# RuyiLian/CheckerPose

Hardware: AMD Instinct MI355X
Metric: crops/sec forward (256x256, npt=512) (higher is better)
Workload: dtype bf16; 1 GPU; LMO 'ape' hr18GNN2_res6_gnn3Skip_mlpQuery npt=512, PoseNet_GNNskip forward, deterministic random-init weights; global_batch=256, parallelism=dp1 (no forward collective), launch=hipGraph replay of 104 kernel launches

## Files before the change

### __graft_entry__.py

```python
import os
import subprocess
import sys

ROOT = os.path.dirname(os.path.abspath(__file__))
if ROOT not in sys.path:
    sys.path.insert(0, ROOT)


def build():
    csrc = os.path.join(ROOT, "checkerpose_amd", "csrc")
    subprocess.check_call(["make", "-C", csrc, "-j4", "ARCH=gfx950"])
    import checkerpose_amd
    from checkerpose_amd import _abi
    lib = _abi.load()
    assert lib.cp_version() >= 232


def smoke():
    import torch
    from oracle import checkerpose_oracle as O
    from checkerpose_amd.synthetic import build_net, det_image
    oracle_kwargs = lambda: dict(backbone="hrnet_w18", res_log2=6, init_n_graph=2, n_graph=3, local_k=2, slope=0.01,
                                 graph_slope=0.2, init_graph_slope=0.2)
    assert torch.cuda.is_available(), "smoke() needs an MI355X"
    torch.set_grad_enabled(False)
    net = build_net(seed=1)
    img = det_image(1, seed=0)
    ref, _ = O.posenet_forward(net.state_dict(), img, net.init_net.knn_idx, 512, **oracle_kwargs())
    net = net.cuda()
    out = net(img.cuda(), None)
# ... 15 lines not shown
```

### checkerpose_amd/_abi.py

```python
import ctypes as C
import os

_HERE = os.path.dirname(os.path.abspath(__file__))
LIB_PATH = os.environ.get("CHECKERPOSE_AMD_LIB") or os.path.join(_HERE, "libcheckerpose_hip.so")

CP_F32, CP_BF16, CP_F16 = 0, 1, 2
ACT_NONE, ACT_RELU, ACT_LEAKY = 0, 1, 2
LOSS_BCE, LOSS_L1 = 0, 1
POSE_ERR_ADD, POSE_ERR_ADI = 1, 2
BOP_ERR_MSSD, BOP_ERR_MSPD, BOP_ERR_PROJ, BOP_MAP_SMALL, BOP_MAP_LARGE = 1, 2, 4, 16, 32
BOP_MATCH_NO_LDS, BOP_MATCH_SCRATCH_MASK, BOP_SCORES_NO_LDS = 1, 2, 1


class CpConvDesc(C.Structure):
    _fields_ = [("dtype", C.c_int32), ("out_f32", C.c_int32), ("B", C.c_int32), ("H", C.c_int32), ("W", C.c_int32),
                ("Cin", C.c_int32), ("in_cstride", C.c_int32), ("in_coff", C.c_int32),
                ("R", C.c_int32), ("S", C.c_int32), ("stride", C.c_int32), ("pad", C.c_int32),
                ("Ho", C.c_int32), ("Wo", C.c_int32), ("Cout", C.c_int32), ("act", C.c_int32), ("slope", C.c_float), ("ksplit", C.c_int32),
                ("o_base", C.c_int64), ("o_sb", C.c_int64), ("o_sy", C.c_int64), ("o_sx", C.c_int64),
                ("o_sc", C.c_int64)]


_P, _I, _F, _L = C.c_void_p, C.c_int, C.c_float, C.c_longlong

# ... 68 lines not shown

SIGNATURES = {
    "cp_version": (_I, []),
    "cp_device_status": (_I, [_P, _I]),
    "cp_set_deterministic": (None, [_I]),
    "cp_get_deterministic": (_I, []),
    "cp_strerror": (C.c_char_p, [_I]),
    "cp_last_kernel": (C.c_char_p, []),
    "cp_kernel_log_begin": (None, []),
    "cp_kernel_log": (C.c_char_p, []),
    "cp_chan_align": (_I, [_I]),
    "cp_packed_weight_bytes": (C.c_size_t, [_I, _I, _I, _I, _I]),
    "cp_pack_conv_weight": (_I, [_P, _I, _P, _I, _I, _I, _I, _I, _I, _I, _P, _I, _P]),
    "cp_conv2d_igemm": (_I, [_P, C.POINTER(CpConvDesc), _P, _P, _P, _P, _P, _P]),
    "cp_conv2d_igemm_splitk": (_I, [_I, C.c_longlong, _I, _I]),
    "cp_packed_halo_weight_bytes": (C.c_size_t, [_I, _I, _I]),
    "cp_pack_conv3x3_halo_weight": (_I, [_P, _I, _P, _I, _I, _I, _P]),
    "cp_conv3x3_halo": (_I, [_P, C.POINTER(CpConvDesc), _P, _P, _P, _P, _P, _P]),
    "cp_conv2x2_halo_supported": (_I, [_I, _I, _I, _I]),
    "cp_packed_conv2x2_halo_weight_bytes": (C.c_size_t, [_I, _I, _I]),
    "cp_pack_conv2x2_halo_weight": (_I, [_P, _I, _P, _I, _I, _I, _P]),
    "cp_conv2x2_halo": (_I, [_P, C.POINTER(CpConvDesc), _P, _P, _P, _P, _P, _P]),
    "cp_conv3x3_s2_small_supported": (_I, [_I, _I, _I, _I]),
    "cp_conv3x3_s2_small_weight_bytes": (C.c_size_t, [_I, _I]),
    "cp_pack_conv3x3_s2_small_weight": (_I, [_P, _P, _I, _I, _I, _I, _P]),
    "cp_conv3x3_s2_small": (_I, [_P, C.POINTER(CpConvDesc), _P, _P, _P, _P, _P]),
    "cp_conv3x3_halo_up2x_supported": (_I, [_I, _I]),
    "cp_conv3x3_halo_up2x": (_I, [_P, C.POINTER(CpConvDesc), _P, _P, _P, _P, _P]),
    "cp_conv3x3_halo_seg_supported": (_I, [_I, _I, _I]),
    "cp_conv3x3_halo_seg": (_I, [_P, C.POINTER(CpConvDesc), _P, _P, _P, _P, _P, _P, _P, _I, _P]),
# ... 270 lines not shown
```

### checkerpose_amd/csrc/api.hip

```cpp
#include <stdarg.h>
#include <stdio.h>
#include <string.h>

#include "common.h"

extern "C" int cp_version(void) { return 232; }

std::atomic<int> g_cp_deterministic{0};
extern "C" void cp_set_deterministic(int on) { g_cp_deterministic.store(on ? 1 : 0, std::memory_order_relaxed); }
extern "C" int cp_get_deterministic(void) { return g_cp_deterministic.load(std::memory_order_relaxed); }

static std::atomic<uint32_t*> g_status_word[256];
uint32_t* cp_status_word(bool create) {
  const int dev = cp_current_device();
  if (dev < 0 || dev > 255) return nullptr;
  uint32_t* p = g_status_word[dev].load(std::memory_order_acquire);
  if (p || !create) return p;
  hipStreamCaptureStatus cs = hipStreamCaptureStatusNone;
  if (hipStreamIsCapturing(nullptr, &cs) == hipSuccess && cs != hipStreamCaptureStatusNone) return nullptr;
  uint32_t* q = nullptr;
  if (hipMalloc((void**)&q, 256) != hipSuccess) return nullptr;
  if (hipMemset(q, 0, 256) != hipSuccess) { (void)hipFree(q); return nullptr; }
  uint32_t* expect = nullptr;
  if (!g_status_word[dev].compare_exchange_strong(expect, q, std::memory_order_acq_rel)) { (void)hipFree(q); return expect; }
// ... 24 lines not shown
  const size_t have = strlen(g_kernel_log);
  if (have + n + 4 < sizeof(g_kernel_log))
    snprintf(g_kernel_log + have, sizeof(g_kernel_log) - have, "%s%s", have ? " + " : "", g_last_kernel);
}
extern "C" const char* cp_last_kernel(void) { return g_last_kernel; }
extern "C" void cp_kernel_log_begin(void) { g_kernel_log[0] = 0; }
extern "C" const char* cp_kernel_log(void) { return g_kernel_log; }

extern "C" const char* cp_strerror(int code) {
  switch (code) {
    case CP_OK: return "ok";
    case CP_ERR_INVALID: return "invalid argument or unsupported shape";
    case CP_ERR_HIP: return "HIP runtime error (kernel launch / graph call failed)";
    case CP_ERR_ALIGN: return "pointer, channel count or stride not aligned to 16 bytes / 4 channels";
    case CP_ERR_RANGE: return "buffer exceeds 2 GiB 32-bit buffer addressing";
    default: return "unknown checkerpose_hip error code";
  }
}

extern "C" int cp_graph_begin_capture(cp_stream_t stream) {
  return hipStreamBeginCapture((hipStream_t)stream, hipStreamCaptureModeThreadLocal) == hipSuccess ? CP_OK : CP_ERR_HIP;
}

extern "C" int cp_graph_end_capture(cp_stream_t stream, void** graph_exec_out) {
  if (!graph_exec_out) return CP_ERR_INVALID;
  hipGraph_t graph = nullptr;
  if (hipStreamEndCapture((hipStream_t)stream, &graph) != hipSuccess || !graph) return CP_ERR_HIP;
  hipGraphExec_t exec = nullptr;
  hipError_t e = hipGraphInstantiate(&exec, graph, nullptr, nullptr, 0);
  (void)hipGraphDestroy(graph);
// ... 15 lines not shown
```

### checkerpose_amd/csrc/conv_igemm.hip

```cpp
#include <stdlib.h>

#include "common.h"

struct ConvParams {
  const void* in; const void* w; const float* scale; const float* shift; const void* res; void* out;
  int M, H, W, HoWo, Wo;
  int Cin, in_cs, in_coff;
  int R, S, stride, pad;
  int KC, Cout, n_tiles, m_blocks, n_blocks, old_map;
  int act; float slope; int out_f32; int epi_lds;
  uint32_t in_bytes, w_bytes;
  long long o_base, o_sb, o_sy, o_sx, o_sc;
};

template <typename Tag> struct Mma;
template <> struct Mma<F32Tag> {
  static __device__ __forceinline__ void run(const u32x4& w, const u32x4& a, f32x4& acc) {
    acc = __builtin_amdgcn_mfma_f32_16x16x4f32(__uint_as_float(w.x), __uint_as_float(a.x), acc, 0, 0, 0);
    acc = __builtin_amdgcn_mfma_f32_16x16x4f32(__uint_as_float(w.y), __uint_as_float(a.y), acc, 0, 0, 0);
    acc = __builtin_amdgcn_mfma_f32_16x16x4f32(__uint_as_float(w.z), __uint_as_float(a.z), acc, 0, 0, 0);
    acc = __builtin_amdgcn_mfma_f32_16x16x4f32(__uint_as_float(w.w), __uint_as_float(a.w), acc, 0, 0, 0);
  }
};
template <> struct Mma<BF16Tag> {
  static __device__ __forceinline__ void run(const u32x4& w, const u32x4& a, f32x4& acc) {
    acc = __builtin_amdgcn_mfma_f32_16x16x32_bf16(__builtin_bit_cast(bf16x8, w), __builtin_bit_cast(bf16x8, a), acc, 0, 0, 0);
  }
};

template <> struct Mma<F16Tag> {
  static __device__ __forceinline__ void run(const u32x4& w, const u32x4& a, f32x4& acc) { acc = cp_mma16<true>(w, a, acc); }
};

template <typename Tag, int MT, int NT>
__global__ __launch_bounds__(256) void conv_igemm_kernel(const ConvParams p) {
  if (p.out_f32 == 2 || Tag::dtype == CP_F16) cp_f16_saturate_on();
  constexpr int E = Tag::E;
  constexpr int KCH = 4 * E;
  constexpr int ES = 16 / E;
  const int lane = threadIdx.x & 63;
  const int wave = __builtin_amdgcn_readfirstlane(threadIdx.x >> 6);
  const int x = lane & 15, q = lane >> 4;
  const int label = blockIdx.x & 7, slot = blockIdx.x >> 3;
  int nblk = slot % p.n_blocks;
  int mblk = (slot / p.n_blocks) * 8 + label;
  if (p.old_map) { const int m8 = (p.m_blocks + 7) / 8 * 8; mblk = blockIdx.x % m8; nblk = blockIdx.x / m8; }
  if (mblk >= p.m_blocks) return;
  const int m_wave = mblk * (4 * MT * 16) + wave * (MT * 16);
  const int nt0 = nblk * NT;

  int iy0[MT], ix0[MT], rowbase[MT];
#pragma unroll
  for (int mt = 0; mt < MT; ++mt) {
    const int m = m_wave + mt * 16 + x;
    const bool ok = m < p.M;
    const int mm = ok ? m : 0;
    const int b = mm / p.HoWo;
    const int rem = mm - b * p.HoWo;
    const int oy = rem / p.Wo;
    const int ox = rem - oy * p.Wo;
    iy0[mt] = ok ? oy * p.stride - p.pad : -(1 << 28);
// ... 218 lines not shown
        for (int j = 0; j < 4; ++j) {
          if (n + j >= p.Cout) continue;
          const long long o = pix[mt] + (long long)(n + j) * p.o_sc;
          float y = v[j];
          if (p.res) y += f32io ? ((const float*)p.res)[o] : bf16_bits_to_f32(((const uint16_t*)p.res)[o]);
          y = cp_act_apply(y, cp_act_slope(p.act, p.slope));
          if (f32io) ((float*)p.out)[o] = y;
          else if (h16out) ((uint16_t*)p.out)[o] = (uint16_t)f32_to_f16_bits_sat(y);
          else ((uint16_t*)p.out)[o] = (uint16_t)f32_to_bf16_bits(y);
        }
      }
    }
  }
}

template <typename Tag, int NT, int KS>
__global__ __launch_bounds__(KS * 64) void conv_igemm_splitk_kernel(const ConvParams p) {
  if (p.out_f32 == 2 || Tag::dtype == CP_F16) cp_f16_saturate_on();
  constexpr int E = Tag::E, KCH = 4 * E, ES = 16 / E, MT = 2, T = MT * NT;
  constexpr int U = NT == 1 ? 8 : (NT == 2 ? 6 : 4);
  __shared__ __attribute__((aligned(16))) float red[KS * T * 64 * 4];
  const int lane = threadIdx.x & 63;
  const int wave = __builtin_amdgcn_readfirstlane(threadIdx.x >> 6);
  const int x = lane & 15, q = lane >> 4;
  const int nblk = blockIdx.x % p.n_blocks, mblk = blockIdx.x / p.n_blocks;
  const int m0 = mblk * (MT * 16), nt0 = nblk * NT;

  int iy0[MT], ix0[MT], rowbase[MT];
#pragma unroll
  for (int mt = 0; mt < MT; ++mt) {
// ... 167 lines not shown
  cp_mark_kernel("conv_igemm_kernel<%s, %d, %d>", Tag::dtype == CP_BF16 ? "BF16Tag" : (Tag::dtype == CP_F16 ? "F16Tag" : "F32Tag"), MT, NT);
  hipLaunchKernelGGL((conv_igemm_kernel<Tag, MT, NT>), grid, dim3(256), lds, st, p);
}

template <typename Tag, int MT>
static void dispatch_nt(const ConvParams& p, int NT, hipStream_t st) {
  switch (NT) {
    case 1: launch<Tag, MT, 1>(p, st); break;
    case 2: launch<Tag, MT, 2>(p, st); break;
    case 3: launch<Tag, MT, 3>(p, st); break;
    case 4: launch<Tag, MT, 4>(p, st); break;
    default: launch<Tag, MT, 5>(p, st); break;
  }
}

extern "C" int cp_conv2d_igemm(cp_stream_t stream, const CpConvDesc* d, const void* in, const void* packed_w,
                               const float* scale, const float* shift, const void* residual, void* out) {
  if (!d || !in || !packed_w || !scale || !shift || !out) return CP_ERR_INVALID;
  if ((d->dtype != CP_F32 && d->dtype != CP_BF16 && d->dtype != CP_F16) || !cp_act_ok(d->act, d->slope)) return CP_ERR_INVALID;
  const bool halfish = d->dtype == CP_F16 || d->out_f32 == 2;
  if (d->out_f32 < 0 || d->out_f32 > 2 || (d->out_f32 == 2 && d->dtype != CP_BF16) || (halfish && residual)) return CP_ERR_INVALID;
  const int E = cp_chan_align(d->dtype), es = cp_elem_size(d->dtype);
  if (d->B <= 0 || d->H <= 0 || d->W <= 0 || d->Ho <= 0 || d->Wo <= 0 || d->R <= 0 || d->S <= 0 || d->stride <= 0)
    return CP_ERR_INVALID;
  if (d->Cin <= 0 || d->Cin % E || d->in_coff % E || d->in_cstride % E || d->in_coff + d->Cin > d->in_cstride)
    return CP_ERR_ALIGN;
  if (d->Cout <= 0 || (d->o_sc == 1 && d->Cout % 4)) return CP_ERR_ALIGN;
  if (!cp_aligned16(in) || !cp_aligned16(packed_w) || !cp_aligned16(scale) || !cp_aligned16(shift))
    return CP_ERR_ALIGN;
  const long long in_bytes = (long long)d->B * d->H * d->W * d->in_cstride * es;
  if (in_bytes >= (1LL << 31)) return CP_ERR_RANGE;
  const long long M = (long long)d->B * d->Ho * d->Wo;
  if (M >= (1LL << 31)) return CP_ERR_RANGE;
  if (d->o_sc == 1) {
    const int oes = d->out_f32 == 1 ? 4 : es;
    if ((d->o_base % 4) || (d->o_sb % 4) || (d->o_sy % 4) || (d->o_sx % 4)) return CP_ERR_ALIGN;
    if (((uintptr_t)out % (4 * oes)) || (residual && ((uintptr_t)residual % (4 * oes)))) return CP_ERR_ALIGN;
  }
  ConvParams p;
  p.in = in; p.w = packed_w; p.scale = scale; p.shift = shift; p.res = residual; p.out = out;
  p.M = (int)M; p.H = d->H; p.W = d->W; p.HoWo = d->Ho * d->Wo; p.Wo = d->Wo;
  p.Cin = d->Cin; p.in_cs = d->in_cstride; p.in_coff = d->in_coff;
  p.R = d->R; p.S = d->S; p.stride = d->stride; p.pad = d->pad;
  const int K = d->R * d->S * d->Cin, KCH = 4 * E;
  p.KC = (K + KCH - 1) / KCH;
  p.Cout = d->Cout; p.n_tiles = (d->Cout + 15) / 16;
  p.act = d->act; p.slope = d->slope; p.out_f32 = d->out_f32;
  p.in_bytes = (uint32_t)in_bytes;
  p.w_bytes = (uint32_t)((size_t)p.n_tiles * p.KC * 1024);
  p.o_base = d->o_base; p.o_sb = d->o_sb; p.o_sy = d->o_sy; p.o_sx = d->o_sx; p.o_sc = d->o_sc;

  int nts = 1;
  if (const int ks = d->ksplit == -1 ? 0 : splitk_plan(d->dtype, M, p.KC, p.n_tiles, &nts)) {
    hipStream_t st_ = (hipStream_t)stream;
    const bool hin = d->dtype == CP_F16;
    if (ks == 8) { if (nts == 3) launch_splitk<3, 8>(p, st_, hin); else if (nts == 2) launch_splitk<2, 8>(p, st_, hin); else launch_splitk<1, 8>(p, st_, hin); }
    else         { if (nts == 3) launch_splitk<3, 4>(p, st_, hin); else if (nts == 2) launch_splitk<2, 4>(p, st_, hin); else launch_splitk<1, 4>(p, st_, hin); }
    return cp_check_launch();
  }
  int NT = 1, best = 1 << 30;
  for (int nt = 5; nt >= 1; --nt) {
    const int padded = (p.n_tiles + nt - 1) / nt * nt;
    if (padded < best) { best = padded; NT = nt; }
  }
  const long long blocks4 = ((M + 255) / 256) * ((p.n_tiles + NT - 1) / NT);
  int MT = (blocks4 >= 512 && p.KC > 4) ? 4 : 2;
  if (const char* e = cp_knob("CP_CONV_MT")) MT = atoi(e) == 2 ? 2 : 4;
  const int oes_ = d->out_f32 == 1 ? 4 : es;
  const int cpl = 16 / oes_;
  p.epi_lds = (MT == 2 && d->o_sc == 1 && !d->out_f32 && !halfish && (NT == 1 || NT == 2 || NT == 4) && d->Cout % cpl == 0 && d->o_base % cpl == 0 &&
               d->o_sb % cpl == 0 && d->o_sy % cpl == 0 && d->o_sx % cpl == 0 && ((uintptr_t)out % 16) == 0 &&
               (!residual || ((uintptr_t)residual % 16) == 0) && !cp_knob("CP_NO_EPI_LDS")) ? 1 : 0;
  hipStream_t st = (hipStream_t)stream;
  if (d->dtype == CP_F32) { if (MT == 4) dispatch_nt<F32Tag, 4>(p, NT, st); else dispatch_nt<F32Tag, 2>(p, NT, st); }
  else if (d->dtype == CP_F16) { if (MT == 4) dispatch_nt<F16Tag, 4>(p, NT, st); else dispatch_nt<F16Tag, 2>(p, NT, st); }
  else                    { if (MT == 4) dispatch_nt<BF16Tag, 4>(p, NT, st); else dispatch_nt<BF16Tag, 2>(p, NT, st); }
  return cp_check_launch();
}
```

### checkerpose_amd/engine.py

```python
import ctypes as C
import os

import torch

from . import _abi
from ._abi import ACT_LEAKY, ACT_NONE, ACT_RELU, CP_BF16, CP_F16, CP_F32, CpChainTail, CpChainTailConv, CpConvDesc, CpFuseConv

_TORCH_DT = {CP_F32: torch.float32, CP_BF16: torch.bfloat16}
USE_HALO = os.environ.get("CHECKERPOSE_AMD_HALO", "1") != "0"
USE_FUSED_BN = os.environ.get("CHECKERPOSE_AMD_FUSED_BN", "1") != "0"
USE_FUSED_BB = os.environ.get("CHECKERPOSE_AMD_FUSED_BB", "1") != "0"
USE_GEMM = os.environ.get("CHECKERPOSE_AMD_GEMM", "1") != "0"
USE_CHAIN = os.environ.get("CHECKERPOSE_AMD_CHAIN", "1") != "0"
USE_UP_FUSED = os.environ.get("CHECKERPOSE_AMD_UP_FUSED", "1") != "0"
USE_FUSE_OUT = os.environ.get("CHECKERPOSE_AMD_FUSE_OUT", "1") != "0"
USE_S2_SMALL = os.environ.get("CHECKERPOSE_AMD_S2_SMALL", "1") != "0"
USE_SEG_FUSED = os.environ.get("CHECKERPOSE_AMD_SEG_FUSED", "1") != "0"
USE_HALO2 = os.environ.get("CHECKERPOSE_AMD_HALO2", "1") != "0"
USE_CHAIN_TAILS = os.environ.get("CHECKERPOSE_AMD_CHAIN_TAILS", "1") != "0"
USE_CHAIN_TAIL = os.environ.get("CHECKERPOSE_AMD_CHAIN_TAIL", "1") != "0"
FUSE_OUT_MIN_BATCH = int(os.environ.get("CHECKERPOSE_AMD_FUSE_OUT_MIN_BATCH", "1"))
USE_MLP_FUSED = os.environ.get("CHECKERPOSE_AMD_MLP_FUSED", "1") != "0"
MLP_FUSED_MIN_ROWS = int(os.environ.get("CHECKERPOSE_AMD_MLP_FUSED_MIN_ROWS", "1"))
EDGE_SCHED = os.environ.get("CHECKERPOSE_AMD_EDGE_SCHED", "1") != "0"
USE_SPLITK = os.environ.get("CHECKERPOSE_AMD_SPLITK", "1") != "0"
GEMM_WS_SMALL_K = os.environ.get("CHECKERPOSE_AMD_GEMM_WS_SMALL_K", "1") != "0"
USE_MLP_GATHER = os.environ.get("CHECKERPOSE_AMD_MLP_GATHER", "1") != "0"
USE_PATCH_GATHER = os.environ.get("CHECKERPOSE_AMD_PATCH_GATHER", "1") != "0"
USE_STEM = os.environ.get("CHECKERPOSE_AMD_STEM", "1") != "0"
STEM_MIN_BATCH = int(os.environ.get("CHECKERPOSE_AMD_STEM_MIN_BATCH", "96"))
USE_EDGE_FUSED = os.environ.get("CHECKERPOSE_AMD_EDGE_FUSED", "1") != "0"
USE_GNN_F16 = os.environ.get("CHECKERPOSE_AMD_GNN_F16", "1") != "0"
USE_EDGE_TILED = os.environ.get("CHECKERPOSE_AMD_EDGE_TILED", "1") != "0"
EDGE_FUSED_MIN_BATCH = int(os.environ.get("CHECKERPOSE_AMD_EDGE_FUSED_MIN_BATCH", "96"))
CHAIN_MIN_BATCH = int(os.environ.get("CHECKERPOSE_AMD_CHAIN_MIN_BATCH", "40"))
NO_RECYCLE = os.environ.get("CHECKERPOSE_AMD_NO_RECYCLE", "0") == "1"
DTYPES = {"fp32": CP_F32, "f32": CP_F32, "float32": CP_F32, "bf16": CP_BF16, "bfloat16": CP_BF16}


class _ConvLog(list):
# ... 213 lines not shown
        return self._nmarks

    def wait(self, token, dst):
        assert self._open is not None
        self.ops.append(("__wait__", token, dst))

    def par_end(self):
        assert self._open is not None
        self.ops.append(("__join__",))
        self.regions.append((self._open - 1, len(self.ops) - 1))
        self._open = None
        self.lane = 0

    def conv(self, x: Act, wkey, w, scale, shift, R, S, stride, pad, Cout, act=ACT_NONE, slope=0.0, residual: Act = None,
             out: Act = None, transposed=0, phase=0, row_map=None, cout_rows=None, out_f32=False, ostr=None,
             out_tbuf=None, out_hw=None, w_shape=None, out_half=False, in_half=False):
        if out_half or in_half:
            assert self.dtype == CP_BF16 and residual is None and not (out_half and out_f32)
        E = self.E
        wCout, wCin = (w.shape[1], w.shape[0]) if transposed else (w.shape[0], w.shape[1])
        rows = cout_rows if cout_rows is not None else wCout
        if wCin != x.C:
            raise RuntimeError("conv %s: weight expects %d input channels, activation has %d" % (wkey, wCin, x.C))
        halo = (USE_HALO and R == 3 and S == 3 and stride == 1 and pad == 1 and ostr is None and not out_f32
                and not transposed and row_map is None and x.W >= 16 and x.H >= 8 and not (out_half or in_half))
        cdt = CP_F16 if in_half else self.dtype
        if halo and wCout <= 80 and self.dtype == CP_F32:
            halo = _rup(x.Cphys, 16) <= 1.15 * x.Cphys
        kmin = 16 * self.E if not (self.dtype == CP_BF16 and residual is None and x.B * x.H * x.W >= 16384 and GEMM_WS_SMALL_K) else 64
        gemm = (USE_GEMM and R == 1 and S == 1 and stride == 1 and pad == 0 and ostr is None and not out_f32
                and not transposed and row_map is None and wCout >= 96 and x.Cphys >= kmin and not out_half)
        s2small = (USE_S2_SMALL and self.dtype == CP_BF16 and R == 3 and S == 3 and stride == 2 and pad == 1 and ostr is None and not out_f32
                   and not transposed and row_map is None and residual is None and x.H % 2 == 0 and x.W % 2 == 0 and x.B >= self.chain_min
                   and not (out_half or in_half) and bool(self.lib.cp_conv3x3_s2_small_supported(x.H, x.W, x.Cphys, _rup(wCout, self.E))))
        halo2 = (USE_HALO2 and self.dtype == CP_BF16 and R == 2 and S == 2 and stride == 1 and pad == 1 and ostr is None and not out_f32
                 and not transposed and row_map is None and not in_half and not self.ws.repacks_every_step
                 and bool(self.lib.cp_conv2x2_halo_supported(self.dtype, x.H, x.W, _rup(wCout, self.E))))
        if (self.splitk and not transposed and row_map is None and (halo or gemm or s2small or halo2)
                and self.lib.cp_conv2d_igemm_splitk(cdt, x.B * ((x.H + 2 * pad - R) // stride + 1) * ((x.W + 2 * pad - S) // stride + 1),
                                                    R * S * x.Cphys, _rup(wCout, self.E))):
            halo = gemm = s2small = halo2 = False
        if s2small:
            packed = self.ws._pack(("s2small", wkey, x.Cphys), self.lib.cp_conv3x3_s2_small_weight_bytes(x.Cphys, _rup(wCout, self.E)), w,
                                   lambda st, wp, op: self.lib.cp_pack_conv3x3_s2_small_weight(st, wp, wCout, wCin, x.Cphys, _rup(wCout, self.E), op),
                                   "cp_pack_conv3x3_s2_small_weight(%s)" % wkey)
            halo = gemm = False
        elif halo2:
            packed = self.ws._pack(("halo2", wkey, x.Cphys), self.lib.cp_packed_conv2x2_halo_weight_bytes(self.dtype, wCout, x.Cphys), w,
                                   lambda st, wp, op: self.lib.cp_pack_conv2x2_halo_weight(st, self.dtype, wp, wCout, wCin, x.Cphys, op),
                                   "cp_pack_conv2x2_halo_weight(%s)" % wkey)
        elif halo:
            packed = self.ws.pack_halo(wkey, w, wCout, wCin, x.Cphys)
        elif gemm:
            packed = self.ws.pack_gemm(wkey, w, wCout, wCin, x.Cphys, **({"dtype": CP_F16} if in_half else {}))
        else:
            packed = self.ws.pack(wkey, w, wCout, wCin, R, S, x.Cphys, rows, transposed, phase, row_map, **({"dtype": CP_F16} if in_half else {}))
# ... 21 lines not shown
        if residual is not None and ostr is None:
            assert (residual.cstride, residual.coff, residual.H, residual.W) == (out.cstride, out.coff, out.H, out.W), \
                "residual must share the output layout"
        fn = self.lib.cp_conv3x3_halo if halo else (self.lib.cp_gemm_rows if gemm else self.lib.cp_conv2d_igemm)
        if halo2:
            fn = self.lib.cp_conv2x2_halo
        dref = C.byref(d)
        pw, ps, pt = packed.data_ptr(), sc.data_ptr(), sh.data_ptr()
        xtb = x.tbuf
        if halo:
            fam = "conv3x3_halo_s" if wCout <= 80 else ("conv3x3_halo4" if wCout % 256 == 0 else "conv3x3_halo")
        else:
            fam = "gemm_rows" if gemm else "conv_igemm"
        if halo2:
            fam = "conv3x3_halo_s"
        if s2small:
            fam = "conv3x3_s2_small"
            self._add(self.lib.cp_conv3x3_s2_small, lambda P: (dref, P(xtb), pw, ps, pt, P(otb)), fam + ":" + wkey, [xtb], [otb])
        else:
            self._add(fn, lambda P: (dref, P(xtb), pw, ps, pt, P(rtb) if rtb is not None else None, P(otb)),
                      fam + ":" + wkey, [xtb, rtb], [otb])
        fl = 2 * x.B * Ho * Wo * R * S * wCin * wCout
        self.flops += fl
        oes = 4 if out_f32 else self.es
        nbytes = (x.B * x.H * x.W * wCin * self.es + x.B * Ho * Wo * wCout * oes * (2 if residual is not None else 1)
                  + R * S * wCin * wCout * self.es)
        self.conv_log.append((wkey, x.B * Ho * Wo, wCout, R * S * wCin, fl, fam, nbytes))
        return out

    def would_splitk(self, M, K, Cout):
        return bool(self.splitk and self.lib.cp_conv2d_igemm_splitk(self.dtype, M, K, _rup(Cout, self.E)))

    def can_conv_up2x(self, H, W, Cout):
        return (USE_UP_FUSED and 2 * H >= 8 and 2 * W >= 16 and
                bool(self.lib.cp_conv3x3_halo_up2x_supported(self.dtype, _rup(Cout, self.E))))

    def conv_up2x(self, x: Act, wkey, w, scale, shift, act=ACT_NONE, slope=0.0, out: Act = None):
        wCout, wCin = w.shape[0], w.shape[1]
        if wCin != x.C:
            raise RuntimeError("conv %s: weight expects %d input channels, activation has %d" % (wkey, wCin, x.C))
        packed = self.ws.pack_halo(wkey, w, wCout, wCin, x.Cphys)
        sc, sh = self.ws.affine(wkey + "#0", scale, shift, wCout)
        Ho, Wo = 2 * x.H, 2 * x.W
# ... 809 lines not shown
```

### checkerpose_amd/netbuilder.py

```python
import os

import torch

from ._abi import ACT_LEAKY, ACT_NONE, ACT_RELU
from .engine import Act, Program, _rup

from .model.backbone import HRNET_CFGS
IMG_FEATS_DIMS = {"resnet34": [64, 128, 256, 512], "hrnet_w18": [128, 256, 512, 1024], "hrnet_w18_small": [128, 256, 512, 1024],
                  "hrnet_w30": [128, 256, 512, 1024]}


FUSE_OUT_DEEP = os.environ.get("CHECKERPOSE_AMD_FUSE_OUT_DEEP", "1") != "0"


DECODER_SPLITK = os.environ.get("CHECKERPOSE_AMD_DECODER_SPLITK", "1") != "0"
HEAD_ON_REFINE_LANE = os.environ.get("CHECKERPOSE_AMD_HEAD_LANE", "1") != "0"
FUSE_SAME_LANE = os.environ.get("CHECKERPOSE_AMD_FUSE_SAME_LANE", "1") != "0"


class NetEmitter:
    def __init__(self, prog: Program, sd):
        self.p, self.ws, self.sd = prog, prog.ws, sd
        self.ones = {}
        self.tp = prog if getattr(prog, "training", False) else None
# ... 633 lines not shown
def _plan_lowcats(em, cfg, active):
    p, nf = em.p, cfg["num_filters"]
    lowcats, feat_outs = {}, None
    if em.tp is None and cfg["backbone"] in HRNET_CFGS:
        feat_outs = [None] * 4
        for i in range(1, active):
            j = 3 - i
            Cs = em.W("init_net.img_backbone.incre_modules.%d.0.conv3.weight" % j).shape[0]
            Hs = cfg["img_size"] // (4 << j)
            if p.can_conv_up2x(Hs, Hs, nf) and not (DECODER_SPLITK and p.would_splitk(p.B * 4 * Hs * Hs, 9 * (_rup(nf, p.E) + _rup(Cs, p.E)), nf)):
                lowcats[i] = p.act(Hs, Hs, nf + Cs)
                feat_outs[j] = lowcats[i].slice(_rup(nf, p.E), Cs)
    return lowcats, feat_outs


def _emit_decoder(em, cfg, io, feats, lowcats, active, after_stage=None):
    p, tp, nf = em.p, em.tp, cfg["num_filters"]
    f = feats[-1]
    cats = {}
    if tp is None:
        for i in range(1, active):
            if i in lowcats:
                continue
            sk = feats[-i - 1]
            cats[i] = p.act(2 * sk.H, 2 * sk.W, nf + sk.C)
            p.set_lane(2)
            p.upsample2x(sk, cats[i].slice(_rup(nf, p.E), sk.C))
    wseg = em.W("seg_block.weight")
    seg_fused = [False]

# ... 2 lines not shown
                and not (DECODER_SPLITK and p.would_splitk(x.B * x.H * x.W, 9 * x.Cphys, em.W(ck + ".weight").shape[0]))):
            s_, t_ = em.ws.bn_fold(bk)
            seg_fused[0] = True
            return p.conv_halo_seg(x, ck, em.W(ck + ".weight"), s_, t_, ACT_RELU, "seg_block", wseg, em.W("seg_block.bias"), io["seg_tb"])
        return em.conv_bn(x, ck, bk, 3, 1, 1, out=out)

    for i in range(active):
        p.set_lane(0)
        up = "up_net.%d" % i
        last = i == active - 1
        nxt = lowcats[i + 1].slice(0, nf) if (i + 1) in lowcats else None
        if i == 0:
            wt = em.W(up + ".0.weight")
            s, t = em.ws.bn_fold(up + ".1") if tp is None else (tp.const_vec(nf, True), tp.const_vec(nf, False))
            o = p.act(2 * f.H, 2 * f.W, nf)
            for ph in range(4):
                a, b = ph >> 1, ph & 1
                if tp is None and ph > 0:
                    p.set_lane(2 + ph)
                p.conv(f, up + ".0", wt, s, t, 1 + a, 1 + b, 1, 0, nf, ACT_RELU if tp is None else ACT_NONE, transposed=1, phase=ph,
                       ostr=((a * o.W + b) * o.cstride, o.H * o.W * o.cstride, 2 * o.W * o.cstride, 2 * o.cstride, 1),
                       out_tbuf=o.tbuf, out_hw=(f.H, f.W))
            if tp is None:
                p.set_lane(0)
                for ph in range(1, 4):
                    p.sync(2 + ph, 0)
            else:
                o = _convt_train_tail(em, up, wt, f, o, nf)
            f = em.conv_bn(o, up + ".3", up + ".4", 3, 1, 1)
            f = tail_conv(f, up + ".6", up + ".7", last, out=nxt)
        elif i in lowcats:
            s1, t1 = em.ws.bn_fold(up + ".2")
            f = p.conv_up2x(lowcats[i], up + ".1", em.W(up + ".1.weight"), s1, t1, ACT_RELU)
            f = tail_conv(f, up + ".4", up + ".5", last, out=nxt)
        else:
            sk = feats[-i - 1]
            cat = cats[i] if i in cats else p.act(2 * f.H, 2 * f.W, f.C + sk.C)
            if i == 1 and i in cats:
                p.sync(2, 0)
            p.upsample2x(f, cat.slice(0, f.C))
            if i not in cats:
                p.upsample2x(sk, cat.slice(f.Cphys, sk.C))
            if tp is not None:
# ... 26 lines not shown
    tp = em.tp

    def local_buf(i):
        gdim = 64 if i == 0 else qd[0]
        return p.act(1, N, qd[0] + gdim)

    L = local_buf(0) if active > 0 else None
    lowcats, feat_outs = _plan_lowcats(em, cfg, active)
    head_later = tp is None and active > 0 and HEAD_ON_REFINE_LANE
    feats, g = emit_init_net(em, cfg, io, "init_net.", graph_out=L.slice(qd[0], 64) if L is not None else None,
                             feat_outs=feat_outs, defer_head=head_later)
    dbits = io.get("decode_bits", io["bits"])
    if not head_later:
        p.decode(dbits, -1, io["mask"], io["xid"], io["yid"], io["x64"], io["y64"], N)
    if active > 0:
        p.par_begin(6 if tp is None else 2)
    if head_later:
        p.set_lane(1)
        g = g()
        p.decode(dbits, -1, io["mask"], io["xid"], io["yid"], io["x64"], io["y64"], N)
        p.set_lane(0)

    def refine(i, f):
        nonlocal L
        p.sync(0, 1)
        p.set_lane(1)
        if tp is None and cfg.get("export_dec"):
            p.to_nchw_f32(f, io["dec_feats"][i])
        if tp is None and cfg.get("inject_dec"):
            t_ = io["inject_dec"][i]
            f = p.nchw_to_nhwc(t_, t_.shape[1], t_.shape[2], t_.shape[3])
# ... 37 lines not shown

def emit_posenet_woprog(em: NetEmitter, cfg, io):
    p = em.p
    N = cfg["npoint"]
    r = cfg["res_log2"]
    nref = r - 3
    active = cfg["stage"] if cfg.get("stage") is not None else nref
    assert 1 <= active <= nref
    ngs = cfg["num_graph_module"]
    ngs = (ngs,) * nref if isinstance(ngs, int) else tuple(ngs)
    slope = cfg["leaky_slope"]
    tp = em.tp
    lowcats, feat_outs = _plan_lowcats(em, cfg, active)
    head_later = tp is None
    feats, g = emit_init_net(em, cfg, io, "init_net.", feat_outs=feat_outs, defer_head=head_later, with_logits=False)
    p.par_begin(6 if tp is None else 2)

    p.set_lane(1)
    if head_later:
        g = g()
    for i in range(active):
        rp = "refine_net.%d" % i
        g = _pre_graph_pair(em, g, rp, slope)
        for gi in range(ngs[i]):
            g = em.edgeconv("%s.pre_query_block.%d" % (rp, gi), g, io["graph"], cfg["graph_slope"])
    if not _query_mlp(em, g, "", slope, io, (0, 13 * N, 0, 1, N), ids=(io["x64"], io["y64"])):
        p.code_decode(io["bits"], 13, r, io["x64"], io["y64"], N)

    p.set_lane(0)
    f = _emit_decoder(em, cfg, io, feats, lowcats, active)
    p.par_end()
# ... 2 lines not shown
```

### include/checkerpose_hip.h

```cpp
#ifndef CHECKERPOSE_HIP_H
#define CHECKERPOSE_HIP_H

#include <stddef.h>
#include <stdint.h>

#ifdef __cplusplus
extern "C" {
#endif

typedef void* cp_stream_t;

enum { CP_F32 = 0, CP_BF16 = 1, CP_F16 = 2 };
enum { CP_ACT_NONE = 0, CP_ACT_RELU = 1, CP_ACT_LEAKY = 2 };
enum { CP_LOSS_BCE = 0, CP_LOSS_L1 = 1 };
enum {
  CP_OK = 0,
  CP_ERR_INVALID = -1,
  CP_ERR_HIP = -2,
  CP_ERR_ALIGN = -3,
  CP_ERR_RANGE = -4
};

int cp_version(void);
const char* cp_strerror(int code);
const char* cp_last_kernel(void);
void cp_kernel_log_begin(void);
const char* cp_kernel_log(void);

void cp_set_deterministic(int on);
int cp_get_deterministic(void);

enum { CP_STATUS_CHAIN0_HANDOVER = 1, CP_STATUS_CHAIN0_STAGING = 2 };
int cp_device_status(uint32_t* status_out, int clear);

int cp_chan_align(int dtype);
// ... 10 lines not shown
  int32_t Cin;
  int32_t in_cstride;
  int32_t in_coff;
  int32_t R, S, stride, pad;
  int32_t Ho, Wo;
  int32_t Cout;
  int32_t act;
  float slope;
  int32_t ksplit;
  int64_t o_base, o_sb, o_sy, o_sx, o_sc;
} CpConvDesc;

int cp_conv2d_igemm(cp_stream_t stream, const CpConvDesc* d, const void* in, const void* packed_w,
                    const float* scale, const float* shift, const void* residual, void* out);
int cp_conv2d_igemm_splitk(int dtype, long long M, int K, int Cout);

size_t cp_packed_halo_weight_bytes(int dtype, int Cout, int cin_phys);
int cp_pack_conv3x3_halo_weight(cp_stream_t stream, int dtype, const float* w, int Cout, int Cin, int cin_phys,
                                void* packed);
int cp_conv3x3_halo(cp_stream_t stream, const CpConvDesc* d, const void* in, const void* packed_w,
                    const float* scale, const float* shift, const void* residual, void* out);
int cp_conv2x2_halo_supported(int dtype, int H, int W, int Cout_phys);
size_t cp_packed_conv2x2_halo_weight_bytes(int dtype, int Cout, int Cin_phys);
int cp_pack_conv2x2_halo_weight(cp_stream_t stream, int dtype, const float* w, int Cout, int Cin, int cin_phys, void* packed);
int cp_conv2x2_halo(cp_stream_t stream, const CpConvDesc* d, const void* in, const void* packed_w, const float* scale,
                    const float* shift, const void* residual, void* out);

int cp_conv3x3_halo_up2x_supported(int dtype, int Cout);
int cp_conv3x3_halo_up2x(cp_stream_t stream, const CpConvDesc* d, const void* in, const void* packed_w,
                         const float* scale, const float* shift, void* out);
// ... 579 lines not shown
```

Baseline: 24880 crops/s.

## Group the four transposed-conv phase GEMMs into one grouped igemm launch

Adds a grouped implicit-GEMM conv kernel that maps one flat grid over up to eight conv problems, each with its own params, and orders members by K depth. The decoder's four transposed-conv phases, previously issued as four launches on separate lanes with syncs, now go out as one launch when all phases share a tile plan. This also reduces the parallel lane count from 6 to 3, cutting launches and cross-stream sync nodes in the graph. In exchange, MT is forced to 2 when phases disagree, and the phases lose any overlap with other lanes that the stream split allowed.

```diff
diff --git a/__graft_entry__.py b/__graft_entry__.py
--- a/__graft_entry__.py
+++ b/__graft_entry__.py
@@ -13,7 +13,7 @@
     import checkerpose_amd
     from checkerpose_amd import _abi
     lib = _abi.load()
-    assert lib.cp_version() >= 232
+    assert lib.cp_version() >= 233
 
 
 def smoke():
diff --git a/checkerpose_amd/_abi.py b/checkerpose_amd/_abi.py
--- a/checkerpose_amd/_abi.py
+++ b/checkerpose_amd/_abi.py
@@ -106,6 +106,8 @@
     "cp_pack_conv_weight": (_I, [_P, _I, _P, _I, _I, _I, _I, _I, _I, _I, _P, _I, _P]),
     "cp_conv2d_igemm": (_I, [_P, C.POINTER(CpConvDesc), _P, _P, _P, _P, _P, _P]),
     "cp_conv2d_igemm_splitk": (_I, [_I, C.c_longlong, _I, _I]),
+    "cp_conv2d_igemm_group": (_I, [_P, _I, C.POINTER(CpConvDesc), _P, _P, _P, _P, _P, _P]),
+    "cp_conv2d_igemm_group_supported": (_I, [_I, C.POINTER(CpConvDesc)]),
     "cp_packed_halo_weight_bytes": (C.c_size_t, [_I, _I, _I]),
     "cp_pack_conv3x3_halo_weight": (_I, [_P, _I, _P, _I, _I, _I, _P]),
     "cp_conv3x3_halo": (_I, [_P, C.POINTER(CpConvDesc), _P, _P, _P, _P, _P, _P]),
diff --git a/checkerpose_amd/csrc/api.hip b/checkerpose_amd/csrc/api.hip
--- a/checkerpose_amd/csrc/api.hip
+++ b/checkerpose_amd/csrc/api.hip
@@ -4,7 +4,7 @@
 
 #include "common.h"
 
-extern "C" int cp_version(void) { return 232; }
+extern "C" int cp_version(void) { return 233; }
 
 std::atomic<int> g_cp_deterministic{0};
 extern "C" void cp_set_deterministic(int on) { g_cp_deterministic.store(on ? 1 : 0, std::memory_order_relaxed); }
@@ -62,6 +62,7 @@
     case CP_ERR_HIP: return "HIP runtime error (kernel launch / graph call failed)";
     case CP_ERR_ALIGN: return "pointer, channel count or stride not aligned to 16 bytes / 4 channels";
     case CP_ERR_RANGE: return "buffer exceeds 2 GiB 32-bit buffer addressing";
+    case CP_ERR_UNSUPPORTED: return "valid arguments this entry point does not take (nothing launched; use the plain entry point)";
     default: return "unknown checkerpose_hip error code";
   }
 }
diff --git a/checkerpose_amd/csrc/conv_igemm.hip b/checkerpose_amd/csrc/conv_igemm.hip
--- a/checkerpose_amd/csrc/conv_igemm.hip
+++ b/checkerpose_amd/csrc/conv_igemm.hip
@@ -33,7 +33,7 @@
 };
 
 template <typename Tag, int MT, int NT>
-__global__ __launch_bounds__(256) void conv_igemm_kernel(const ConvParams p) {
+__device__ __forceinline__ void conv_igemm_body(const ConvParams p, int block_in_member) {
   if (p.out_f32 == 2 || Tag::dtype == CP_F16) cp_f16_saturate_on();
   constexpr int E = Tag::E;
   constexpr int KCH = 4 * E;
@@ -41,10 +41,11 @@
   const int lane = threadIdx.x & 63;
   const int wave = __builtin_amdgcn_readfirstlane(threadIdx.x >> 6);
   const int x = lane & 15, q = lane >> 4;
-  const int label = blockIdx.x & 7, slot = blockIdx.x >> 3;
+  const unsigned bim = (unsigned)block_in_member;
+  const int label = bim & 7, slot = bim >> 3;
   int nblk = slot % p.n_blocks;
   int mblk = (slot / p.n_blocks) * 8 + label;
-  if (p.old_map) { const int m8 = (p.m_blocks + 7) / 8 * 8; mblk = blockIdx.x % m8; nblk = blockIdx.x / m8; }
+  if (p.old_map) { const int m8 = (p.m_blocks + 7) / 8 * 8; mblk = bim % m8; nblk = bim / m8; }
   if (mblk >= p.m_blocks) return;
   const int m_wave = mblk * (4 * MT * 16) + wave * (MT * 16);
   const int nt0 = nblk * NT;
@@ -293,6 +294,27 @@
   }
 }
 
+template <typename Tag, int MT, int NT>
+__global__ __launch_bounds__(256) void conv_igemm_kernel(const ConvParams p) {
+  conv_igemm_body<Tag, MT, NT>(p, (int)blockIdx.x);
+}
+
+#define CP_CONV_GROUP_MAX 8
+struct ConvGroupParams {
+  ConvParams m[CP_CONV_GROUP_MAX];
+  int first[CP_CONV_GROUP_MAX + 1];
+  int n;
+};
+
+template <typename Tag, int MT, int NT>
+__global__ __launch_bounds__(256) void conv_igemm_group_kernel(const ConvGroupParams g) {
+  const int blk = (int)blockIdx.x;
+  int i = 0;
+#pragma unroll
+  for (int k = 1; k < CP_CONV_GROUP_MAX; ++k) i += (k < g.n && blk >= g.first[k]) ? 1 : 0;
+  conv_igemm_body<Tag, MT, NT>(g.m[i], blk - g.first[i]);
+}
+
 template <typename Tag, int NT, int KS>
 __global__ __launch_bounds__(KS * 64) void conv_igemm_splitk_kernel(const ConvParams p) {
   if (p.out_f32 == 2 || Tag::dtype == CP_F16) cp_f16_saturate_on();
@@ -490,9 +512,9 @@
   }
 }
 
-extern "C" int cp_conv2d_igemm(cp_stream_t stream, const CpConvDesc* d, const void* in, const void* packed_w,
-                               const float* scale, const float* shift, const void* residual, void* out) {
-  if (!d || !in || !packed_w || !scale || !shift || !out) return CP_ERR_INVALID;
+static int conv_prepare(const CpConvDesc* d, const void* in, const void* packed_w, const float* scale, const float* shift,
+                        const void* residual, void* out, bool ptrs, ConvParams* p_, long long* M_) {
+  if (!d || (ptrs && (!in || !packed_w || !scale || !shift || !out))) return CP_ERR_INVALID;
   if ((d->dtype != CP_F32 && d->dtype != CP_BF16 && d->dtype != CP_F16) || !cp_act_ok(d->act, d->slope)) return CP_ERR_INVALID;
   const bool halfish = d->dtype == CP_F16 || d->out_f32 == 2;
   if (d->out_f32 < 0 || d->out_f32 > 2 || (d->out_f32 == 2 && d->dtype != CP_BF16) || (halfish && residual)) return CP_ERR_INVALID;
@@ -502,7 +524,7 @@
   if (d->Cin <= 0 || d->Cin % E || d->in_coff % E || d->in_cstride % E || d->in_coff + d->Cin > d->in_cstride)
     return CP_ERR_ALIGN;
   if (d->Cout <= 0 || (d->o_sc == 1 && d->Cout % 4)) return CP_ERR_ALIGN;
-  if (!cp_aligned16(in) || !cp_aligned16(packed_w) || !cp_aligned16(scale) || !cp_aligned16(shift))
+  if (ptrs && (!cp_aligned16(in) || !cp_aligned16(packed_w) || !cp_aligned16(scale) || !cp_aligned16(shift)))
     return CP_ERR_ALIGN;
   const long long in_bytes = (long long)d->B * d->H * d->W * d->in_cstride * es;
   if (in_bytes >= (1LL << 31)) return CP_ERR_RANGE;
@@ -511,9 +533,10 @@
   if (d->o_sc == 1) {
     const int oes = d->out_f32 == 1 ? 4 : es;
     if ((d->o_base % 4) || (d->o_sb % 4) || (d->o_sy % 4) || (d->o_sx % 4)) return CP_ERR_ALIGN;
-    if (((uintptr_t)out % (4 * oes)) || (residual && ((uintptr_t)residual % (4 * oes)))) return CP_ERR_ALIGN;
-  }
-  ConvParams p;
+    if (ptrs && (((uintptr_t)out % (4 * oes)) || (residual && ((uintptr_t)residual % (4 * oes))))) return CP_ERR_ALIGN;
+  }
+  ConvParams& p = *p_;
+  p = ConvParams{};
   p.in = in; p.w = packed_w; p.scale = scale; p.shift = shift; p.res = residual; p.out = out;
   p.M = (int)M; p.H = d->H; p.W = d->W; p.HoWo = d->Ho * d->Wo; p.Wo = d->Wo;
   p.Cin = d->Cin; p.in_cs = d->in_cstride; p.in_coff = d->in_coff;
@@ -525,7 +548,36 @@
   p.in_bytes = (uint32_t)in_bytes;
   p.w_bytes = (uint32_t)((size_t)p.n_tiles * p.KC * 1024);
   p.o_base = d->o_base; p.o_sb = d->o_sb; p.o_sy = d->o_sy; p.o_sx = d->o_sx; p.o_sc = d->o_sc;
-
+  *M_ = M;
+  return CP_OK;
+}
+
+static void conv_tiles(const ConvParams& p, long long M, int* NT_, int* MT_) {
+  int NT = 1, best = 1 << 30;
+  for (int nt = 5; nt >= 1; --nt) {
+    const int padded = (p.n_tiles + nt - 1) / nt * nt;
+    if (padded < best) { best = padded; NT = nt; }
+  }
+  const long long blocks4 = ((M + 255) / 256) * ((p.n_tiles + NT - 1) / NT);
+  int MT = (blocks4 >= 512 && p.KC > 4) ? 4 : 2;
+  if (const char* e = cp_knob("CP_CONV_MT")) MT = atoi(e) == 2 ? 2 : 4;
+  *NT_ = NT; *MT_ = MT;
+}
+
+static int conv_epi_lds(const CpConvDesc* d, int MT, int NT, const void* out, const void* residual) {
+  const bool halfish = d->dtype == CP_F16 || d->out_f32 == 2;
+  const int oes_ = d->out_f32 == 1 ? 4 : cp_elem_size(d->dtype);
+  const int cpl = 16 / oes_;
+  return (MT == 2 && d->o_sc == 1 && !d->out_f32 && !halfish && (NT == 1 || NT == 2 || NT == 4) && d->Cout % cpl == 0 && d->o_base % cpl == 0 &&
+          d->o_sb % cpl == 0 && d->o_sy % cpl == 0 && d->o_sx % cpl == 0 && ((uintptr_t)out % 16) == 0 &&
+          (!residual || ((uintptr_t)residual % 16) == 0) && !cp_knob("CP_NO_EPI_LDS")) ? 1 : 0;
+}
+
+extern "C" int cp_conv2d_igemm(cp_stream_t stream, const CpConvDesc* d, const void* in, const void* packed_w,
+                               const float* scale, const float* shift, const void* residual, void* out) {
+  ConvParams p;
+  long long M = 0;
+  if (const int rc = conv_prepare(d, in, packed_w, scale, shift, residual, out, true, &p, &M)) return rc;
   int nts = 1;
   if (const int ks = d->ksplit == -1 ? 0 : splitk_plan(d->dtype, M, p.KC, p.n_tiles, &nts)) {
     hipStream_t st_ = (hipStream_t)stream;
@@ -534,22 +586,101 @@
     else         { if (nts == 3) launch_splitk<3, 4>(p, st_, hin); else if (nts == 2) launch_splitk<2, 4>(p, st_, hin); else launch_splitk<1, 4>(p, st_, hin); }
     return cp_check_launch();
   }
-  int NT = 1, best = 1 << 30;
-  for (int nt = 5; nt >= 1; --nt) {
-    const int padded = (p.n_tiles + nt - 1) / nt * nt;
-    if (padded < best) { best = padded; NT = nt; }
-  }
-  const long long blocks4 = ((M + 255) / 256) * ((p.n_tiles + NT - 1) / NT);
-  int MT = (blocks4 >= 512 && p.KC > 4) ? 4 : 2;
-  if (const char* e = cp_knob("CP_CONV_MT")) MT = atoi(e) == 2 ? 2 : 4;
-  const int oes_ = d->out_f32 == 1 ? 4 : es;
-  const int cpl = 16 / oes_;
-  p.epi_lds = (MT == 2 && d->o_sc == 1 && !d->out_f32 && !halfish && (NT == 1 || NT == 2 || NT == 4) && d->Cout % cpl == 0 && d->o_base % cpl == 0 &&
-               d->o_sb % cpl == 0 && d->o_sy % cpl == 0 && d->o_sx % cpl == 0 && ((uintptr_t)out % 16) == 0 &&
-               (!residual || ((uintptr_t)residual % 16) == 0) && !cp_knob("CP_NO_EPI_LDS")) ? 1 : 0;
+  int NT, MT;
+  conv_tiles(p, M, &NT, &MT);
+  p.epi_lds = conv_epi_lds(d, MT, NT, out, residual);
   hipStream_t st = (hipStream_t)stream;
   if (d->dtype == CP_F32) { if (MT == 4) dispatch_nt<F32Tag, 4>(p, NT, st); else dispatch_nt<F32Tag, 2>(p, NT, st); }
   else if (d->dtype == CP_F16) { if (MT == 4) dispatch_nt<F16Tag, 4>(p, NT, st); else dispatch_nt<F16Tag, 2>(p, NT, st); }
   else                    { if (MT == 4) dispatch_nt<BF16Tag, 4>(p, NT, st); else dispatch_nt<BF16Tag, 2>(p, NT, st); }
   return cp_check_launch();
 }
+
+struct ConvGroupPlan {
+  ConvGroupParams g;
+  int NT, MT;
+  size_t lds;
+};
+
+static int conv_group_plan(int n, const CpConvDesc* descs, const void* const* ins, const void* const* ws, const float* const* scales,
+                           const float* const* shifts, const void* const* residuals, void* const* outs, bool ptrs, ConvGroupPlan* plan) {
+  if (n < 1 || n > CP_CONV_GROUP_MAX || !descs || (ptrs && (!ins || !ws || !scales || !shifts || !outs))) return CP_ERR_INVALID;
+  ConvParams ps[CP_CONV_GROUP_MAX];
+  int NT = 0, MT = 0;
+  bool mt_agree = true;
+  for (int i = 0; i < n; ++i) {
+    const CpConvDesc* d = descs + i;
+    const void* res = (ptrs && residuals) ? residuals[i] : nullptr;
+    long long M = 0;
+    if (const int rc = conv_prepare(d, ptrs ? ins[i] : nullptr, ptrs ? ws[i] : nullptr, ptrs ? scales[i] : nullptr,
+                                    ptrs ? shifts[i] : nullptr, res, ptrs ? outs[i] : nullptr, ptrs, &ps[i], &M)) return rc;
+    if (res || d->dtype == CP_F16 || d->out_f32 == 2 || d->dtype != descs[0].dtype) return CP_ERR_UNSUPPORTED;
+    int nts = 1;
+    if (d->ksplit != -1 && splitk_plan(d->dtype, M, ps[i].KC, ps[i].n_tiles, &nts)) return CP_ERR_UNSUPPORTED;
+    int nt, mt;
+    conv_tiles(ps[i], M, &nt, &mt);
+    if (i == 0) { NT = nt; MT = mt; }
+    if (nt != NT) return CP_ERR_UNSUPPORTED;
+    mt_agree = mt_agree && mt == MT;
+  }
+  if (cp_knob("CP_NO_CONV_GROUP")) return CP_ERR_UNSUPPORTED;
+  if (!mt_agree) MT = 2;
+  int order[CP_CONV_GROUP_MAX];
+  for (int i = 0; i < n; ++i) order[i] = i;
+  for (int i = 1; i < n; ++i)
+    for (int j = i; j > 0 && ps[order[j]].KC > ps[order[j - 1]].KC; --j) { const int t = order[j]; order[j] = order[j - 1]; order[j - 1] = t; }
+  ConvGroupParams& g = plan->g;
+  g = ConvGroupParams{};
+  g.n = n;
+  long long first = 0;
+  size_t lds = 0;
+  for (int k = 0; k < n; ++k) {
+    const int i = order[k];
+    ConvParams& p = g.m[k];
+    p = ps[i];
+    p.m_blocks = (p.M + 4 * MT * 16 - 1) / (4 * MT * 16);
+    p.n_blocks = (p.n_tiles + NT - 1) / NT;
+    p.old_map = cp_knob("CP_OLD_MAP") ? 1 : 0;
+    p.epi_lds = ptrs ? conv_epi_lds(descs + i, MT, NT, outs[i], nullptr) : 0;
+    if (p.epi_lds) lds = (size_t)4 * MT * 16 * (NT * 16 + 4) * sizeof(float);
+    g.first[k] = (int)first;
+    first += (long long)((p.m_blocks + 7) / 8 * 8) * p.n_blocks;
+    if (first >= (1LL << 31)) return CP_ERR_RANGE;
+  }
+  for (int k = n; k <= CP_CONV_GROUP_MAX; ++k) g.first[k] = (int)first;
+  plan->NT = NT; plan->MT = MT; plan->lds = lds;
+  return CP_OK;
+}
+
+template <typename Tag, int MT, int NT>
+static void launch_group(const ConvGroupPlan& pl, hipStream_t st) {
+  cp_mark_kernel("conv_igemm_group_kernel<%s, %d, %d>", Tag::dtype == CP_BF16 ? "BF16Tag" : "F32Tag", MT, NT);
+  hipLaunchKernelGGL((conv_igemm_group_kernel<Tag, MT, NT>), dim3((unsigned)pl.g.first[pl.g.n]), dim3(256), pl.lds, st, pl.g);
+}
+
+template <typename Tag, int MT>
+static void dispatch_group_nt(const ConvGroupPlan& pl, hipStream_t st) {
+  switch (pl.NT) {
+    case 1: launch_group<Tag, MT, 1>(pl, st); break;
+    case 2: launch_group<Tag, MT, 2>(pl, st); break;
+    case 3: launch_group<Tag, MT, 3>(pl, st); break;
+    case 4: launch_group<Tag, MT, 4>(pl, st); break;
+    default: launch_group<Tag, MT, 5>(pl, st); break;
+  }
+}
+
+extern "C" int cp_conv2d_igemm_group_supported(int n, const CpConvDesc* descs) {
+  ConvGroupPlan pl;
+  return conv_group_plan(n, descs, nullptr, nullptr, nullptr, nullptr, nullptr, nullptr, false, &pl);
+}
+
+extern "C" int cp_conv2d_igemm_group(cp_stream_t stream, int n, const CpConvDesc* descs, const void* const* ins, const void* const* ws,
+                                     const float* const* scales, const float* const* shifts, const void* const* residuals,
+                                     void* const* outs) {
+  ConvGroupPlan pl;
+  if (const int rc = conv_group_plan(n, descs, ins, ws, scales, shifts, residuals, outs, true, &pl)) return rc;
+  hipStream_t st = (hipStream_t)stream;
+  if (descs[0].dtype == CP_F32) { if (pl.MT == 4) dispatch_group_nt<F32Tag, 4>(pl, st); else dispatch_group_nt<F32Tag, 2>(pl, st); }
+  else                          { if (pl.MT == 4) dispatch_group_nt<BF16Tag, 4>(pl, st); else dispatch_group_nt<BF16Tag, 2>(pl, st); }
+  return cp_check_launch();
+}
diff --git a/checkerpose_amd/engine.py b/checkerpose_amd/engine.py
--- a/checkerpose_amd/engine.py
+++ b/checkerpose_amd/engine.py
@@ -24,6 +24,8 @@
 MLP_FUSED_MIN_ROWS = int(os.environ.get("CHECKERPOSE_AMD_MLP_FUSED_MIN_ROWS", "1"))
 EDGE_SCHED = os.environ.get("CHECKERPOSE_AMD_EDGE_SCHED", "1") != "0"
 USE_SPLITK = os.environ.get("CHECKERPOSE_AMD_SPLITK", "1") != "0"
+USE_CONVT_GROUP = os.environ.get("CHECKERPOSE_AMD_CONVT_GROUP", "1") != "0"
+CONV_GROUP_MAX = 8
 GEMM_WS_SMALL_K = os.environ.get("CHECKERPOSE_AMD_GEMM_WS_SMALL_K", "1") != "0"
 USE_MLP_GATHER = os.environ.get("CHECKERPOSE_AMD_MLP_GATHER", "1") != "0"
 USE_PATCH_GATHER = os.environ.get("CHECKERPOSE_AMD_PATCH_GATHER", "1") != "0"
@@ -267,7 +269,7 @@
 
     def conv(self, x: Act, wkey, w, scale, shift, R, S, stride, pad, Cout, act=ACT_NONE, slope=0.0, residual: Act = None,
              out: Act = None, transposed=0, phase=0, row_map=None, cout_rows=None, out_f32=False, ostr=None,
-             out_tbuf=None, out_hw=None, w_shape=None, out_half=False, in_half=False):
+             out_tbuf=None, out_hw=None, w_shape=None, out_half=False, in_half=False, _member=None):
         if out_half or in_half:
             assert self.dtype == CP_BF16 and residual is None and not (out_half and out_f32)
         E = self.E
@@ -293,6 +295,10 @@
                 and self.lib.cp_conv2d_igemm_splitk(cdt, x.B * ((x.H + 2 * pad - R) // stride + 1) * ((x.W + 2 * pad - S) // stride + 1),
                                                     R * S * x.Cphys, _rup(wCout, self.E))):
             halo = gemm = s2small = halo2 = False
+        if _member is not None and (halo or gemm or s2small or halo2 or residual is not None or out_half or in_half
+                                    or (ostr is None and out is None)):
+            _member.append(None)
+            return None
         if s2small:
             packed = self.ws._pack(("s2small", wkey, x.Cphys), self.lib.cp_conv3x3_s2_small_weight_bytes(x.Cphys, _rup(wCout, self.E)), w,
                                    lambda st, wp, op: self.lib.cp_pack_conv3x3_s2_small_weight(st, wp, wCout, wCin, x.Cphys, _rup(wCout, self.E), op),
@@ -344,19 +350,53 @@
             fam = "gemm_rows" if gemm else "conv_igemm"
         if halo2:
             fam = "conv3x3_halo_s"
+        fl = 2 * x.B * Ho * Wo * R * S * wCin * wCout
+        oes = 4 if out_f32 else self.es
+        nbytes = (x.B * x.H * x.W * wCin * self.es + x.B * Ho * Wo * wCout * oes * (2 if residual is not None else 1)
+                  + R * S * wCin * wCout * self.es)
+        if _member is not None:
+            _member.append((d, xtb, pw, ps, pt, otb, (wkey, x.B * Ho * Wo, wCout, R * S * wCin, fl, fam, nbytes)))
+            return out
         if s2small:
             fam = "conv3x3_s2_small"
             self._add(self.lib.cp_conv3x3_s2_small, lambda P: (dref, P(xtb), pw, ps, pt, P(otb)), fam + ":" + wkey, [xtb], [otb])
         else:
             self._add(fn, lambda P: (dref, P(xtb), pw, ps, pt, P(rtb) if rtb is not None else None, P(otb)),
                       fam + ":" + wkey, [xtb, rtb], [otb])
-        fl = 2 * x.B * Ho * Wo * R * S * wCin * wCout
-        self.flops += fl
-        oes = 4 if out_f32 else self.es
-        nbytes = (x.B * x.H * x.W * wCin * self.es + x.B * Ho * Wo * wCout * oes * (2 if residual is not None else 1)
-                  + R * S * wCin * wCout * self.es)
+        self.flops += fl
         self.conv_log.append((wkey, x.B * Ho * Wo, wCout, R * S * wCin, fl, fam, nbytes))
         return out
+
+    def _group_members(self, members):
+        if not (USE_CONVT_GROUP and 1 <= len(members) <= CONV_GROUP_MAX):
+            return None
+        recs = []
+        for m in members:
+            self.conv(_member=recs, **m)
+            if recs[-1] is None:
+                return None
+        descs = (CpConvDesc * len(recs))(*[r[0] for r in recs])
+        if self.lib.cp_conv2d_igemm_group_supported(len(recs), descs) != 0:
+            return None
+        return recs, descs
+
+    def can_conv_group(self, members):
+        return self._group_members(members) is not None
+
+    def conv_group(self, members):
+        recs, descs = self._group_members(members)
+        n = len(recs)
+        arr = lambda vals: (C.c_void_p * n)(*vals)
+        pws, pss, pts = arr([r[2] for r in recs]), arr([r[3] for r in recs]), arr([r[4] for r in recs])
+        xtbs, otbs = [r[1] for r in recs], [r[5] for r in recs]
+        self.keep += [descs, pws, pss, pts]
+        log = [r[6] for r in recs]
+        self._add(self.lib.cp_conv2d_igemm_group,
+                  lambda P: (n, descs, arr([P(t) for t in xtbs]), pws, pss, pts, None, arr([P(t) for t in otbs])),
+                  "conv_igemm:%s#group%d" % (log[0][0], n), xtbs, otbs)
+        fl = sum(e[4] for e in log)
+        self.flops += fl
+        self.conv_log.append((log[0][0], sum(e[1] for e in log), log[0][2], max(e[3] for e in log), fl, "conv_igemm", sum(e[6] for e in log)))
 
     def would_splitk(self, M, K, Cout):
         return bool(self.splitk and self.lib.cp_conv2d_igemm_splitk(self.dtype, M, K, _rup(Cout, self.E)))
diff --git a/checkerpose_amd/netbuilder.py b/checkerpose_amd/netbuilder.py
--- a/checkerpose_amd/netbuilder.py
+++ b/checkerpose_amd/netbuilder.py
@@ -671,6 +671,27 @@
     return lowcats, feat_outs
 
 
+def _convt_phases(em, f, o, s, t):
+    tp, nf = em.tp, o.C
+    return [dict(x=f, wkey="up_net.0.0", w=em.W("up_net.0.0.weight"), scale=s, shift=t, R=1 + (ph >> 1), S=1 + (ph & 1), stride=1, pad=0,
+                 Cout=nf, act=ACT_RELU if tp is None else ACT_NONE, transposed=1, phase=ph,
+                 ostr=(((ph >> 1) * o.W + (ph & 1)) * o.cstride, o.H * o.W * o.cstride, 2 * o.W * o.cstride, 2 * o.cstride, 1),
+                 out_tbuf=o.tbuf, out_hw=(f.H, f.W)) for ph in range(4)]
+
+
+def _decoder_lanes(em, cfg, f, active):
+    if em.tp is not None:
+        return 2
+    p, nf = em.p, cfg["num_filters"]
+    if active > 0:
+        cp_ = _rup(nf, p.E)
+        o = Act(None, f.B, 2 * f.H, 2 * f.W, nf, cp_, cp_, 0)
+        s, t = em.ws.bn_fold("up_net.0.1")
+        if p.can_conv_group(_convt_phases(em, f, o, s, t)):
+            return 3
+    return 6
+
+
 def _emit_decoder(em, cfg, io, feats, lowcats, active, after_stage=None):
     p, tp, nf = em.p, em.tp, cfg["num_filters"]
     f = feats[-1]
@@ -703,19 +724,20 @@
             wt = em.W(up + ".0.weight")
             s, t = em.ws.bn_fold(up + ".1") if tp is None else (tp.const_vec(nf, True), tp.const_vec(nf, False))
             o = p.act(2 * f.H, 2 * f.W, nf)
-            for ph in range(4):
-                a, b = ph >> 1, ph & 1
-                if tp is None and ph > 0:
-                    p.set_lane(2 + ph)
-                p.conv(f, up + ".0", wt, s, t, 1 + a, 1 + b, 1, 0, nf, ACT_RELU if tp is None else ACT_NONE, transposed=1, phase=ph,
-                       ostr=((a * o.W + b) * o.cstride, o.H * o.W * o.cstride, 2 * o.W * o.cstride, 2 * o.cstride, 1),
-                       out_tbuf=o.tbuf, out_hw=(f.H, f.W))
-            if tp is None:
-                p.set_lane(0)
-                for ph in range(1, 4):
-                    p.sync(2 + ph, 0)
+            phases = _convt_phases(em, f, o, s, t)
+            if tp is None and p.can_conv_group(phases):
+                p.conv_group(phases)
             else:
-                o = _convt_train_tail(em, up, wt, f, o, nf)
+                for ph in range(4):
+                    if tp is None and ph > 0:
+                        p.set_lane(2 + ph)
+                    p.conv(**phases[ph])
+                if tp is None:
+                    p.set_lane(0)
+                    for ph in range(1, 4):
+                        p.sync(2 + ph, 0)
+                else:
+                    o = _convt_train_tail(em, up, wt, f, o, nf)
             f = em.conv_bn(o, up + ".3", up + ".4", 3, 1, 1)
             f = tail_conv(f, up + ".6", up + ".7", last, out=nxt)
         elif i in lowcats:
@@ -772,7 +794,7 @@
     if not head_later:
         p.decode(dbits, -1, io["mask"], io["xid"], io["yid"], io["x64"], io["y64"], N)
     if active > 0:
-        p.par_begin(6 if tp is None else 2)
+        p.par_begin(_decoder_lanes(em, cfg, feats[-1], active))
     if head_later:
         p.set_lane(1)
         g = g()
@@ -840,7 +862,7 @@
     lowcats, feat_outs = _plan_lowcats(em, cfg, active)
     head_later = tp is None
     feats, g = emit_init_net(em, cfg, io, "init_net.", feat_outs=feat_outs, defer_head=head_later, with_logits=False)
-    p.par_begin(6 if tp is None else 2)
+    p.par_begin(_decoder_lanes(em, cfg, feats[-1], active))
 
     p.set_lane(1)
     if head_later:
diff --git a/include/checkerpose_hip.h b/include/checkerpose_hip.h
--- a/include/checkerpose_hip.h
+++ b/include/checkerpose_hip.h
@@ -18,7 +18,8 @@
   CP_ERR_INVALID = -1,
   CP_ERR_HIP = -2,
   CP_ERR_ALIGN = -3,
-  CP_ERR_RANGE = -4
+  CP_ERR_RANGE = -4,
+  CP_ERR_UNSUPPORTED = -5
 };
 
 int cp_version(void);
@@ -59,6 +60,9 @@
 int cp_conv2d_igemm(cp_stream_t stream, const CpConvDesc* d, const void* in, const void* packed_w,
                     const float* scale, const float* shift, const void* residual, void* out);
 int cp_conv2d_igemm_splitk(int dtype, long long M, int K, int Cout);
+int cp_conv2d_igemm_group(cp_stream_t stream, int n, const CpConvDesc* descs, const void* const* ins, const void* const* ws,
+                          const float* const* scales, const float* const* shifts, const void* const* residuals, void* const* outs);
+int cp_conv2d_igemm_group_supported(int n, const CpConvDesc* descs);
 
 size_t cp_packed_halo_weight_bytes(int dtype, int Cout, int cin_phys);
 int cp_pack_conv3x3_halo_weight(cp_stream_t stream, int dtype, const float* w, int Cout, int Cin, int cin_phys,
```

Result: no change. 24710 crops/s (-0.7%).
